# ZencashOfficial/ginger-lib

Hardware: AMD Instinct MI355X
Metric: MNT4-753 G1 MSM scalar-muls/sec + 2^n NTT ms at 1/2/4/8 MI355X (higher is better)
Workload: dtype u32 (29-bit limbs of 753-bit Montgomery residues, 64-bit accumulators)

## Files before the change

ginger-lib_amd/asmgen/build.py:

```python
import json
import os
import subprocess
import sys

from . import g1_reduce, g1_xyzz, g2_rounds, microbench, ntt_pass
from .isa import module_text

LLVM = os.environ.get("GH_LLVM_BIN", "/opt/rocm/lib/llvm/bin")

P4 = 0x1c4c62d92c41110229022eee2cdadb7f997505b8fafed5eb7e8f96c97d87307fdb925e8a0ed8d99d124d9a15af79db117e776f218059db80f0da5cb537e38685acce9767254a4638810719ac425f0e39d54522cdd119f5e9063de245e8001
P6 = 0x1c4c62d92c41110229022eee2cdadb7f997505b8fafed5eb7e8f96c97d87307fdb925e8a0ed8d99d124d9a15af79db26c5c28c859a99b3eebca9429212636b9dff97634993aa4d6c381bc3f0057974ea099170fa13a4fd90776e240000001
R = 1 << 754


def programs():
    progs = [
        g1_xyzz.build("gh_asm_acc_g1_p4", P4, R % P4),
        g1_xyzz.build("gh_asm_acc_g1_p6", P6, R % P6),
        g1_xyzz.build("gh_asm_acc_g1_p4_pw", P4, R % P4, persistent=True),
        g1_xyzz.build("gh_asm_acc_g1_p6_pw", P6, R % P6, persistent=True),
        g1_reduce.build("gh_asm_red_g1_p4", P4, R % P4),
        g1_reduce.build("gh_asm_red_g1_p6", P6, R % P6),
    ]
    c2 = g2_rounds.Cfg(2, 13, P4, R % P4)
    c3 = g2_rounds.Cfg(3, 11, P6, R % P6)
    c1a = g2_rounds.Cfg(1, 1, P4, R % P4)
    c1b = g2_rounds.Cfg(1, 1, P6, R % P6)
    for tag, cfg in (("f2", c2), ("f3", c3), ("f1p4", c1a), ("f1p6", c1b)):
        for fwd in (True, False):
            for r0 in (True, False):
                progs.append(g2_rounds.build("gh_asm_aff_%s_%s_%s" % (tag, "fwd" if fwd else "bwd", "r0" if r0 else "rn"), cfg, fwd, r0))
    for tag, prime in (("p4", P4), ("p6", P6)):
        for k in (6, 7, 8):
            progs.append(ntt_pass.build("gh_asm_ntt_%s_k%d" % (tag, k), prime, k))
    progs.append(microbench.build("gh_asm_mb_mulpair", P4))
    if os.environ.get("GH_ASM_DEBUG"):
        progs.append(g2_rounds.build("gh_asm_aff_f2_bwd_r0_dbg", c2, False, True, debug=True))
        for tag, prime in (("p4", P4), ("p6", P6)):
            progs.append(g1_xyzz.build("gh_asm_acc_g1_%s_dbg" % tag, prime, R % prime, debug=True))
            progs.append(g1_xyzz.build("gh_asm_acc_g1_%s_pw_dbg" % tag, prime, R % prime, persistent=True, debug=True))
    if os.environ.get("GH_ASM_VARIANTS"):
        progs += [g1_xyzz.build("gh_asm_acc_g1_p4_s1", P4, R % P4, split=1),
                  g1_xyzz.build("gh_asm_acc_g1_p4_s2", P4, R % P4, split=2),
                  g1_xyzz.build("gh_asm_acc_g1_p4_s1pf", P4, R % P4, split=1, prefetch=True)]
    return progs


def build(outdir):
    os.makedirs(outdir, exist_ok=True)
# ... 1 lines not shown
    text, infos = module_text(progs)
    s_path = os.path.join(outdir, "gh_asm.s")
    with open(s_path, "w") as f:
        f.write(text)
    o_path = os.path.join(outdir, "gh_asm.o")
    co_path = os.path.join(outdir, "gh_asm.hsaco")
    subprocess.run([os.path.join(LLVM, "clang"), "-x", "assembler", "-target", "amdgcn-amd-amdhsa", "-mcpu=gfx950",
                    "-c", s_path, "-o", o_path], check=True)
    subprocess.run([os.path.join(LLVM, "ld.lld"), "-shared", o_path, "-o", co_path], check=True)
    for p in progs:
        infos[p.name]["instructions"] = p.count()
        infos[p.name]["lds_bytes"] = p.lds_bytes
        infos[p.name]["scratch_bytes_per_lane"] = 0
        if getattr(p, "loop_labels", None):
            infos[p.name].update(g1_xyzz.update_counts(p))
    with open(os.path.join(outdir, "gh_asm.json"), "w") as f:
        json.dump(infos, f, indent=1, sort_keys=True)
    return co_path, infos


if __name__ == "__main__":
    co, infos = build(sys.argv[1] if len(sys.argv) > 1 else "build")
    print(co, json.dumps(infos))
```

ginger-lib_amd/asmgen/field.py:

```python
from .isa import Reg, V, S

NL = 26
LB = 29
LM = (1 << LB) - 1


ND = NL + 1
TOP_SHIFT = LB * (NL - 1)


class BoundError(ValueError):
    """a lazy routine was asked for operands whose columns, top limb or doubled limb do not fit the registers"""


class Bound:

    def __init__(self, k, slack=0):
        self.k, self.slack = k, slack

    def value(self, p):
        return self.k * p + self.slack

    def __repr__(self):
        return "Bound(%d p + 2^%.1f)" % (self.k, _log2(self.slack)) if self.slack else "Bound(%d p)" % self.k
# ... 428 lines not shown
            o = dst.sub(i) if i == NL - 1 else x
            if a is None:
                if i:
                    g.v_add_u32(o, t, c); yield
                else:
                    g.v_mov_b32(o, t); yield
            elif i:
                g.v_add3_u32(o, t, a.sub(i), c); yield
            else:
                g.v_add_u32(o, t, a.sub(0)); yield
            if i + 1 < NL:
                g.v_ashrrev_i32(c, LB, x); yield
                g.v_and_b32(dst.sub(i), S(self.s_lm), x); yield
        return res

    def zero_or_p_mask(self, ch, a, smask, stmp):
        g = self.g
        skip = g.uniq("zp_skip")
        g.v_cmp_eq_u32(smask, 0, a.sub(0))
        g.v_cmp_eq_u32(stmp, self.sP(0), a.sub(0))
        g.s_or_b64(smask, smask, stmp)
        g.s_cbranch_scc0(skip)
        run(self.is_zero_mask(ch, a, smask))
        x = ch.acc.lo()
        g.v_xor_b32(x, self.sP(0), a.sub(0))
        for i in range(1, NL):
            g.v_xor_b32(ch.t1, self.sP(i), a.sub(i))
            g.v_or_b32(x, x, ch.t1)
        g.v_cmp_eq_u32(stmp, 0, x)
        g.s_or_b64(smask, smask, stmp)
# ... 35 lines not shown
```

ginger-lib_amd/asmgen/ntt_pass.py:

```python
from .isa import Prog, V, S, VCC, EXEC, OFF, fix_hazards
from .field import FieldGen, Chain, run, NL, LB, LM

ARG_IN, ARG_OUT, ARG_TW, ARG_PRE, ARG_POST = 0, 8, 16, 24, 32
ARG_LOGN, ARG_LOGNS, ARG_INVERSE, ARG_POST_STRIDE, ARG_NWAVES = 40, 44, 48, 52, 56
ARG_BYTES = 64

S_KARG, S_WG = S(0, 2), S(2)
S_IN, S_OUT, S_TW, S_PRE, S_POST = S(4, 2), S(6, 2), S(8, 2), S(10, 2), S(12, 2)
S_LOGN, S_LOGNS, S_INVERSE, S_PSTRIDE, S_NWAVES = S(14), S(15), S(16), S(17), S(18)
S_LM, S_INV = 20, 21
S_P, S_NP = 24, 50
S_DUM, S_CAR, S_MASK = S(22, 2), S(76, 2), S(78, 2)
S_SSH, S_SH, S_NMASK, S_N, S_NSMASK, S_96, S_104, S_WAVE, S_T0, S_T1 = (S(80), S(81), S(82), S(83), S(84), S(85), S(86), S(87),
                                                                         S(88), S(89))

V_TID, V_LANE, V_TL, V_J, V_KK = V(0), V(1), V(2), V(3), V(4)
V_OFF = [V(5), V(6), V(7), V(8)]
V_IDX = [V(9), V(10), V(11), V(12)]
V_T = [V(13), V(14), V(15), V(16), V(17), V(18), V(19)]


def slot(i):
    return V(20 + NL * i, NL)


E = [slot(i) for i in range(4)]
TWA, TWB, M, D = slot(4), slot(5), slot(6), slot(7)
STAGE = [TWA, TWB, M, D]


def build(name, p, k):
    assert 4 <= k <= 8
    log_c = 8 - k
    g = Prog(name)
    for _ in range(5):
        g.add_arg(8, "ptr")
    for _ in range(6):
        g.add_arg(4, "val")
    assert g.kernarg_bytes == ARG_BYTES
    f = FieldGen(g, p, S_P, S_NP, S_INV, S_LM)
    ch = Chain(V(228, 2), V(230), V(231), S_DUM, S_CAR)
    L_END, L_GO = g.uniq("end"), g.uniq("go")

    def load_fp(dst, voff, sbase):
        for q in range(NL // 2):
            g.global_load_dwordx2(V(dst.idx + 2 * q, 2), voff, sbase, offset=8 * q)
# ... 29 lines not shown
                prev = w
            if lo + 1 < NL:
                g.v_lshl_or_b32(w, src.sub(lo + 1), LB - sh, prev)
                prev = w
            if lo + 2 < NL and 2 * LB - sh < 32:
                g.v_lshl_or_b32(w, src.sub(lo + 2), 2 * LB - sh, prev)
                prev = w
            assert prev is w

    def tw_offset(dst, e):
        g.v_sub_u32(V_T[6], S_N, e)
        g.v_and_b32(V_T[6], S_NMASK, V_T[6])
        g.v_cndmask_b32(dst, e, V_T[6], S_T0X)
        g.v_mul_lo_u32(dst, dst, S_104)

    def butterfly(x, y, tw):
        if tw is None:
            run(f.sub(ch, x, y, D))
            run(f.add_mod(ch, x, y))
            run(f.copy(y, D))
        else:
            run(f.mul(ch, y, tw, M, D, dst=D))
            run(f.sub(ch, x, D, y))
            run(f.add_mod(ch, x, D))

    def times(x, tw):
        run(f.mul(ch, x, tw, M, tw, dst=x))

    S_T0X = S(90, 2)

    g.s_load_dwordx8(S(4, 8), S_KARG, 0)
    g.s_load_dwordx8(S(12, 8), S_KARG, 32)
    f.load_constants()
    g.s_mov_b32(S_96, 96)
    g.s_mov_b32(S_104, 104)
    g.v_and_b32(V_LANE, 63, V_TID)
    g.v_lshrrev_b32(V_T[0], 6, V_TID)
    g.v_readfirstlane_b32(S_WAVE, V_T[0])
    g.s_lshl_b32(S_T0, S_WG, 2)
    g.s_add_u32(S_WAVE, S_WAVE, S_T0)
    g.s_waitcnt(lgkmcnt=0)
    g.s_cmp_lt_u32(S_WAVE, S_NWAVES)
    g.s_cbranch_scc1(L_GO)
    g.s_endpgm()
    g.label(L_GO)
    g.s_sub_u32(S_SSH, S_LOGN, k)
    g.s_sub_u32(S_SH, S_SSH, S_LOGNS)
    g.s_lshl_b32(S_N, 1, S_LOGN)
# ... 20 lines not shown
        load_raw(STAGE[a], V_OFF[a])
    for a in range(4):
        g.s_waitcnt(vmcnt=6 * (3 - a))
        unpack(E[a], STAGE[a])

    L_NOPRE = g.uniq("nopre")
    S_JMP = S(92, 2)
    g.s_cmp_eq_u64(S_PRE, 0)
    g.s_cbranch_scc0(g_pre := g.uniq("pre"))
    g.long_branch(L_NOPRE, S_JMP)
    g.label(g_pre)
    for a in range(4):
        g.v_mul_lo_u32(V_OFF[a], V_IDX[a], S_104)
    load_fp(TWA, V_OFF[0], S_PRE)
    for a in range(4):
        cur, nxt = (TWA, TWB) if a % 2 == 0 else (TWB, TWA)
        if a + 1 < 4:
            load_fp(nxt, V_OFF[a + 1], S_PRE)
            g.s_waitcnt(vmcnt=NL // 2)
        else:
            g.s_waitcnt(vmcnt=0)
        times(E[a], cur)
    g.label(L_NOPRE)


    inl = [k - 2, k - 1]
    V_BP, V_E, V_REV = V_T[4], V_T[5], V_T[3]
    S_T2 = S(94)
    g.v_bfrev_b32(V_REV, V_TL)
    g.v_lshrrev_b32(V_REV, 32 - (k - 2), V_REV)
    for beta in range(k - 1, -1, -1):
        last = beta == 0
        if beta in inl:
            b = inl.index(beta)
            swap_q = None
        else:
            b = 0 if inl[0] > inl[1] else 1
            swap_q = beta + log_c
        pairs = [(0, 2), (1, 3)] if b == 1 else [(0, 1), (2, 3)]
        g.s_add_u32(S_T1, S_SH, beta)
        g.s_add_u32(S_T2, S_SSH, beta)
        g.v_lshlrev_b32(V_E, S_T1, V_KK)
        tws = [TWA]
        if beta <= k - 2:
            nrev = k - 2 - beta
            if nrev > 0:
                g.v_and_b32(V_T[0], (1 << nrev) - 1, V_REV)
# ... 24 lines not shown
            inl[b] = beta
        g.s_waitcnt(vmcnt=0)
        for n, (x, y) in enumerate(pairs):
            tw = tws[min(n, len(tws) - 1)]
            if beta == k - 1 or (beta == k - 2 and n == 0):
                L_FULL, L_NEXT = g.uniq("full"), g.uniq("next")
                g.s_cmp_eq_u32(S_LOGNS, 0)
                g.s_cbranch_scc0(L_FULL)
                butterfly(E[x], E[y], None)
                g.long_branch(L_NEXT, S_JMP)
                g.label(L_FULL)
                butterfly(E[x], E[y], tw)
                g.label(L_NEXT)
            else:
                butterfly(E[x], E[y], tw)
    g.v_sub_u32(V_T[0], V_J, V_KK)
    g.v_lshlrev_b32(V_T[0], k, V_T[0])
    g.v_add_u32(V_T[0], V_T[0], V_KK)
    g.v_lshlrev_b32(V_T[1], 2, V_TL)
    g.v_bfrev_b32(V_T[1], V_T[1])
    g.v_lshrrev_b32(V_T[1], 32 - k, V_T[1])
    for a in range(4):
        t_low = (((a >> 0) & 1) << inl[0]) | (((a >> 1) & 1) << inl[1])
        rev = int(format(t_low, "0%db" % k)[::-1], 2)
        g.v_or_b32(V_IDX[a], rev, V_T[1])
        g.v_lshlrev_b32(V_IDX[a], S_LOGNS, V_IDX[a])
        g.v_add_u32(V_IDX[a], V_IDX[a], V_T[0])
    L_STORE = g.uniq("store")
    g.s_cmp_eq_u64(S_POST, 0)
    g.s_cbranch_scc0(g_post := g.uniq("post"))
    g.long_branch(L_STORE, S_JMP)
    g.label(g_post)
    for a in range(4):
        g.v_mul_lo_u32(V_OFF[a], V_IDX[a], S_PSTRIDE)
    load_fp(TWA, V_OFF[0], S_POST)
    for a in range(4):
        cur, nxt = (TWA, TWB) if a % 2 == 0 else (TWB, TWA)
        if a + 1 < 4:
            load_fp(nxt, V_OFF[a + 1], S_POST)
            g.s_waitcnt(vmcnt=NL // 2)
        else:
            g.s_waitcnt(vmcnt=0)
        times(E[a], cur)
    g.label(L_STORE)
    for a in range(4):
        g.v_mul_lo_u32(V_OFF[a], V_IDX[a], S_96)
    for a in range(4):
        pack(STAGE[a], E[a])
        for q in range(6):
            g.global_store_dwordx4(V_OFF[a], V(STAGE[a].idx + 4 * q, 4), S_OUT, offset=16 * q)
    g.s_endpgm()
    g.label(L_END)
    g.s_endpgm()
    g.hazard_nops = fix_hazards(g)
    return g
```

ginger-lib_amd/csrc/asm_kernels.h:

```cpp
#pragma once
#include "runtime.h"

namespace gh_asm {

struct AccTask {
    uint32_t beg, cnt;
    uint64_t dst;
};
static_assert(sizeof(AccTask) == 16, "the kernel reads one dwordx4 per task");

bool enabled();

int acc_g1_launch(int prime, const void* bases, const uint32_t* sorted, const AccTask* tasks, const void* salts,
                  uint32_t n_tasks, uint32_t* tile_counter, hipStream_t st);
int acc_stamps_read(uint32_t* out_words, size_t cap_words, uint32_t* n_records);

struct RedArgs {
    const void* items;
    void* out;
    void* slabs;
    uint32_t* flag;
    uint32_t count, valid, segs, L, n_programs, pad;
};
static_assert(sizeof(RedArgs) == 56, "argument block of gh_asm_red_g1_*");
// ... 15 lines not shown
};
static_assert(sizeof(AffArgs) == 88, "argument block of gh_asm_aff_*");

bool aff_enabled();
bool aff_g1_enabled();
int aff_launch(int kind, bool fwd, bool r0, const AffArgs& a, uint32_t waves, hipStream_t st);

struct NttAsmArgs {
    const void* in;
    void* out;
    const void* tw;
    const void* pre;
    const void* post;
    uint32_t log_n, log_ns, inverse;
    uint32_t post_stride;
    uint32_t n_waves, pad;
};
static_assert(sizeof(NttAsmArgs) == 64, "argument block of gh_asm_ntt_*");

bool ntt_enabled();
bool ntt_supported(int log_n, int k);
int ntt_pass_launch(int prime, int k, const NttAsmArgs& a, hipStream_t st);

int measure_fpmul_peak(double* products_per_s, hipStream_t st);
int kernel_resources(const char* which, uint32_t* scratch, uint32_t* vgprs, uint32_t* lds);

}
```

ginger-lib_amd/csrc/asm_kernels.hip:

```cpp
#include "asm_kernels.h"
#include <stdio.h>
#include <stdlib.h>
#include <string.h>
#include <vector>

extern "C" const unsigned char gh_asm_hsaco[];
extern "C" const unsigned char gh_asm_hsaco_end[];

namespace gh_asm {

using gh_rt::g;
using gh_rt::g_err;
using gh_rt::env_int;

namespace {
constexpr int NTT_ASM_KMIN = 6, NTT_ASM_KMAX = 8;
struct State {
    bool tried = false;
    hipModule_t mod = nullptr;
    hipFunction_t acc_g1[2] = {nullptr, nullptr};
    hipFunction_t acc_g1_pw[2] = {nullptr, nullptr};
    hipFunction_t acc_g1_dbg[2][2] = {};
    uint32_t* stamps[2] = {nullptr, nullptr};
    size_t stamps_cap[2] = {0, 0};
    uint32_t stamps_n = 0;
    int stamps_last = 1;
    hipFunction_t red_g1[2] = {nullptr, nullptr};
    hipFunction_t aff[4][2][2] = {};
    hipFunction_t mb_mulpair = nullptr;
    hipFunction_t ntt[2][3] = {};
};
State s;

int load_locked() {
    if (s.tried) return s.mod ? GH_OK : GH_E_HIP;
    s.tried = true;
    const size_t bytes = (size_t)(gh_asm_hsaco_end - gh_asm_hsaco);
    if (bytes < 64 || memcmp(gh_asm_hsaco, "\177ELF", 4) != 0) {
        g_err = "assembly code object missing from the library (build/gh_asm.hsaco was not embedded)";
        return GH_E_HIP;
    }
    hipModule_t m = nullptr;
    hipError_t e;
    static std::vector<char> override_co;
    if (const char* path = getenv("GH_ASM_HSACO")) {
// ... 51 lines not shown
        }
    }
    static const char* kinds[4] = {"f2", "f3", "f1p4", "f1p6"};
    for (int t = 0; t < 4; t++)
        for (int fw = 0; fw < 2; fw++)
            for (int r0 = 0; r0 < 2; r0++) {
                char nm[64];
                snprintf(nm, sizeof nm, "gh_asm_aff_%s_%s_%s", kinds[t], fw ? "fwd" : "bwd", r0 ? "r0" : "rn");
                e = hipModuleGetFunction(&s.aff[t][fw][r0], m, nm);
                if (e != hipSuccess) {
                    g_err = std::string("hipModuleGetFunction(") + nm + ") failed: " + hipGetErrorString(e);
                    hipModuleUnload(m);
                    return GH_E_HIP;
                }
            }
    for (int f = 0; f < 2; f++)
        for (int k = NTT_ASM_KMIN; k <= NTT_ASM_KMAX; k++) {
            char nm[64];
            snprintf(nm, sizeof nm, "gh_asm_ntt_p%d_k%d", f ? 6 : 4, k);
            e = hipModuleGetFunction(&s.ntt[f][k - NTT_ASM_KMIN], m, nm);
            if (e != hipSuccess) {
                g_err = std::string("hipModuleGetFunction(") + nm + ") failed: " + hipGetErrorString(e);
                hipModuleUnload(m);
                return GH_E_HIP;
            }
        }
    e = hipModuleGetFunction(&s.mb_mulpair, m, "gh_asm_mb_mulpair");
    if (e != hipSuccess) {
        g_err = std::string("hipModuleGetFunction(gh_asm_mb_mulpair) failed: ") + hipGetErrorString(e);
        hipModuleUnload(m);
        return GH_E_HIP;
    }
    s.mod = m;
    g.at_shutdown.push_back([] {
        if (s.mod) hipModuleUnload(s.mod);
        for (uint32_t* b : s.stamps) if (b) (void)hipFree(b);
        s = State();
    });
    return GH_OK;
}
}
// ... 126 lines not shown
        return GH_E_UNSUPPORTED;
    }
    if (int rc = load_locked()) return rc;
    AffArgs args = a;
    size_t size = sizeof args;
    void* extra[] = {HIP_LAUNCH_PARAM_BUFFER_POINTER, &args, HIP_LAUNCH_PARAM_BUFFER_SIZE, &size, HIP_LAUNCH_PARAM_END};
    HIPCHK(hipModuleLaunchKernel(s.aff[tower][fwd ? 1 : 0][r0 ? 1 : 0], waves / 4, 1, 1, 256, 1, 1, 0, st, nullptr, extra));
    return GH_OK;
}

bool ntt_enabled() {
    static const bool on = env_int("GH_NTT_ASM", 1) != 0;
    return on;
}

bool ntt_supported(int log_n, int k) { return k >= NTT_ASM_KMIN && k <= NTT_ASM_KMAX && log_n >= 8 && log_n <= 25 && k <= log_n; }

int ntt_pass_launch(int prime, int k, const NttAsmArgs& a, hipStream_t st) {
    if (!ntt_supported((int)a.log_n, k) || a.log_ns + (uint32_t)k > a.log_n || a.n_waves != (1u << (a.log_n - 8)) ||
        (a.post_stride != 0 && a.post_stride != 104)) {
        g_err = "internal: NTT pass outside the assembly kernel's range";
        return GH_E_UNSUPPORTED;
    }
    if (int rc = load_locked()) return rc;
    NttAsmArgs args = a;
    size_t size = sizeof args;
    void* extra[] = {HIP_LAUNCH_PARAM_BUFFER_POINTER, &args, HIP_LAUNCH_PARAM_BUFFER_SIZE, &size, HIP_LAUNCH_PARAM_END};
    HIPCHK(hipModuleLaunchKernel(s.ntt[prime == 6 ? 1 : 0][k - NTT_ASM_KMIN], (a.n_waves + 3) / 4, 1, 1, 256, 1, 1, 0, st, nullptr, extra));
    return GH_OK;
}

int measure_fpmul_peak(double* products_per_s, hipStream_t st) {
    if (int rc = load_locked()) return rc;
    const uint32_t iters = 200, blocks = (uint32_t)g.num_cus * 2u;
    struct { uint32_t iters, pad; } args = {iters, 0};
    size_t size = sizeof args;
    void* extra[] = {HIP_LAUNCH_PARAM_BUFFER_POINTER, &args, HIP_LAUNCH_PARAM_BUFFER_SIZE, &size, HIP_LAUNCH_PARAM_END};
    hipEvent_t e0, e1;
    HIPCHK(hipEventCreate(&e0));
    HIPCHK(hipEventCreate(&e1));
    float best = 0;
    for (int rep = 0; rep < 4; rep++) {
        HIPCHK(hipEventRecord(e0, st));
// ... 14 lines not shown
    if (int rc = load_locked()) return rc;
    hipFunction_t f = nullptr;
    const std::string w = which ? which : "";
    if (w == "g1_acc_p4") f = s.acc_g1[0];
    else if (w == "g1_acc_p6") f = s.acc_g1[1];
    else if (w == "g1_acc_p4_pw") f = s.acc_g1_pw[0];
    else if (w == "g1_acc_p6_pw") f = s.acc_g1_pw[1];
    else if (w == "g1_red_p4") f = s.red_g1[0];
    else if (w == "g1_red_p6") f = s.red_g1[1];
    else if (w == "g2_f2_fwd_r0") f = s.aff[0][1][1];
    else if (w == "g2_f2_bwd_r0") f = s.aff[0][0][1];
    else if (w == "g2_f2_bwd_rn") f = s.aff[0][0][0];
    else if (w == "g2_f3_fwd_r0") f = s.aff[1][1][1];
    else if (w == "g2_f3_bwd_r0") f = s.aff[1][0][1];
    else if (w == "g2_f3_bwd_rn") f = s.aff[1][0][0];
    else if (w == "ntt_p4_k8") f = s.ntt[0][2];
    else if (w == "ntt_p6_k8") f = s.ntt[1][2];
    else { g_err = "unknown kernel name"; return GH_E_BAD_ARG; }
    int v = 0;
    HIPCHK(hipFuncGetAttribute(&v, HIP_FUNC_ATTRIBUTE_LOCAL_SIZE_BYTES, f));
    if (scratch) *scratch = (uint32_t)v;
    HIPCHK(hipFuncGetAttribute(&v, HIP_FUNC_ATTRIBUTE_NUM_REGS, f));
    if (vgprs) *vgprs = (uint32_t)v;
    HIPCHK(hipFuncGetAttribute(&v, HIP_FUNC_ATTRIBUTE_SHARED_SIZE_BYTES, f));
    if (lds) *lds = (uint32_t)v;
    return GH_OK;
}

}
```

ginger-lib_amd/csrc/fp29.h:

```cpp
#pragma once
#include <stdint.h>
#include "constants_gen.h"

#if defined(__HIPCC__)
#define GH_HD __host__ __device__ __forceinline__
#define GH_HD_NOINLINE __host__ __device__ __attribute__((noinline))
#define GH_UNROLL _Pragma("unroll")
#else
#define GH_HD inline
#define GH_HD_NOINLINE __attribute__((noinline))
#define GH_UNROLL
#endif

namespace gh {

constexpr int NL = 26;
constexpr int LB = 29;
constexpr uint32_t LM = (1u << LB) - 1;

struct Fp {
    uint32_t l[NL];
};

struct P4 {
// ... 370 lines not shown
template <class P> GH_HD bool fp_is_zero_or_p(const Fp& a) {
    if (a.l[0] != 0 && a.l[0] != P::P[0]) return false;
    uint32_t z = 0, e = 0;
    GH_UNROLL for (int i = 0; i < NL; i++) {
        z |= a.l[i];
        e |= a.l[i] ^ P::P[i];
    }
    return z == 0 || e == 0;
}
template <class P> GH_HD Fp fp_lazy_one() {
    Fp d3 = fp_zero();
    d3.l[3] = 1;
    Fp c = fp_mul27<P>(fp_const<P>(P::R2I), d3);
    fp_cond_sub<P>(c);
    return c;
}

constexpr int FP_INV_BATCHES = 61;

template <class P> GH_HD Fp fp_inv_plain(const Fp& x) {
    int32_t d[NL], e[NL], f[NL], g[NL];
    GH_UNROLL for (int i = 0; i < NL; i++) { d[i] = 0; e[i] = 0; f[i] = (int32_t)P::P[i]; g[i] = (int32_t)x.l[i]; }
    e[0] = 1;
    int32_t zeta = -1;
    const uint32_t pinv = (0u - P::INV) & LM;
#if defined(__HIP_DEVICE_COMPILE__)
#pragma nounroll
#endif
    for (int it = 0; it < FP_INV_BATCHES; it++) {
        uint32_t u = 1, v = 0, q = 0, r = 1, fl = (uint32_t)f[0], gl = (uint32_t)g[0];
// ... 244 lines not shown
```

ginger-lib_amd/csrc/ntt.hip:

```cpp
#include "runtime.h"
#include "ntt_kernels.h"
#include "host_math.h"
#include "asm_kernels.h"

namespace gh_rt {
using namespace gh;

template <class P> struct FieldConsts;
template <> struct FieldConsts<P6> {
    static constexpr int two_adicity = GH_P6_TWO_ADICITY;
    static const uint64_t* root_m() { static const uint64_t v[12] = GH_P6_ROOT_M_64; return v; }
    static const uint64_t* gen_m() { static const uint64_t v[12] = GH_P6_GEN17_M_64; return v; }
};
template <> struct FieldConsts<P4> {
    static constexpr int two_adicity = GH_P4_TWO_ADICITY;
    static const uint64_t* root_m() { static const uint64_t v[12] = GH_P4_ROOT_M_64; return v; }
    static const uint64_t* gen_m() { static const uint64_t v[12] = GH_P4_GEN17_M_64; return v; }
};

template <class P> int build_pow_table(Fp* tab, int log_n, const Fp& first, Fp base) {
    HIPCHK(hipMemcpyAsync(tab, &first, sizeof(Fp), hipMemcpyHostToDevice, g.stream));
    HIPCHK(hipStreamSynchronize(g.stream));
    for (int s = 0; s < log_n; s++) {
        uint32_t half = 1u << s;
        hipLaunchKernelGGL((pow_table_step_kernel<P>), dim3((half + 255) / 256), dim3(256), 0, g.stream, tab, half, base);
        base = fp_sqr<P>(base);
    }
    HIPCHK(hipGetLastError());
    return GH_OK;
}

template <class P> int build_table_checked(DevMem& t, int log_n, const Fp& first, const Fp& base) {
    int rc;
    if ((rc = t.alloc(((size_t)1 << log_n) * sizeof(Fp))) || (rc = build_pow_table<P>(t.as<Fp>(), log_n, first, base))) return rc;
    if (hipStreamSynchronize(g.stream) != hipSuccess) { g_err = "building a domain table failed"; return GH_E_HIP; }
    return GH_OK;
}

template <class P> int get_domain(int fidx, int log_n, bool need_coset, bool need_coset_inv, Domain** out) {
    auto it = g.domains[fidx].find(log_n);
    const size_t N = (size_t)1 << log_n;
    if (it == g.domains[fidx].end()) {
        Domain d;
        d.log_n = log_n;
        Fp w = fp_from_abi<P>(reinterpret_cast<const uint32_t*>(FieldConsts<P>::root_m()));
        for (int i = log_n; i < FieldConsts<P>::two_adicity; i++) w = fp_sqr<P>(w);
        Fp n_int = fp_one<P>();
        for (int i = 0; i < log_n; i++) n_int = fp_dbl<P>(n_int);
        d.size_inv = host_fp_inv<P>(n_int);
        DevMem scratch, tw, size_inv;
        int rc;
        if ((rc = scratch.alloc(N * 96)) || (rc = build_table_checked<P>(tw, log_n, fp_one<P>(), w)) || (rc = size_inv.alloc(128))) return rc;
        HIPCHK(hipMemcpy(size_inv.get(), &d.size_inv, sizeof(Fp), hipMemcpyHostToDevice));
        d.scratch = (uint32_t*)scratch.release();
        d.tw = (Fp*)tw.release();
        d.d_size_inv = (Fp*)size_inv.release();
        it = g.domains[fidx].emplace(log_n, d).first;
    }
    Domain& d = it->second;
    if (need_coset && !d.coset) {
        Fp gen = fp_from_abi<P>(reinterpret_cast<const uint32_t*>(FieldConsts<P>::gen_m()));
        DevMem t;
        if (int rc = build_table_checked<P>(t, log_n, fp_one<P>(), gen)) return rc;
        d.coset = (Fp*)t.release();
    }
    if (need_coset_inv && !d.coset_inv) {
        Fp gen = fp_from_abi<P>(reinterpret_cast<const uint32_t*>(FieldConsts<P>::gen_m()));
        Fp gi = host_fp_inv<P>(gen);
        DevMem t;
        if (int rc = build_table_checked<P>(t, log_n, d.size_inv, gi)) return rc;
        d.coset_inv = (Fp*)t.release();
    }
    *out = &d;
    return GH_OK;
}

template <class P> int fft_run(int fidx, void* d_data, uint32_t log_n, uint32_t flags, bool sync = true) {
    if ((int)log_n >= FieldConsts<P>::two_adicity) {
        g_err = "domain exceeds the field's 2-adicity";
        return GH_E_UNSUPPORTED;
    }
    g.last_fft_ms = 0;
    if (log_n == 0) return GH_OK;
    const bool inverse = flags & GH_FFT_INVERSE, coset = flags & GH_FFT_COSET;
    Domain* d;
    int rc = get_domain<P>(fidx, (int)log_n, coset && !inverse, coset && inverse, &d);
    if (rc) return rc;
    const int P_ = ((int)log_n + NTT_MAX_LOGR - 1) / NTT_MAX_LOGR;
    int ks[8];
    {
        int base = (int)log_n / P_, rem = (int)log_n % P_;
        for (int s = 0; s < P_; s++) ks[s] = base + (s < rem ? 1 : 0);
    }
    static bool attr_set[2] = {false, false};
    if (!attr_set[fidx]) {
        HIPCHK(hipFuncSetAttribute(reinterpret_cast<const void*>(&ntt_pass_kernel<P>),
                                   hipFuncAttributeMaxDynamicSharedMemorySize, NL * 4 * NTT_MAX_TILE));
        attr_set[fidx] = true;
    }
    if (P_ >= 3 && (P_ & 1) && !d->scratch2 && !d->scratch2_failed) {
        DevMem s2;
        if (s2.alloc(((size_t)96) << log_n)) {
            (void)hipGetLastError();
            d->scratch2_failed = true;
        }
        d->scratch2 = (uint32_t*)s2.release();
    }
    const bool three = P_ >= 3 && (P_ & 1) && d->scratch2;
    uint32_t* bufs[2] = {(uint32_t*)d_data, d->scratch};
    int cur = 0, log_ns = 0;
    static const bool ntt_asm = gh_asm::ntt_enabled();
    HIPCHK(hipEventRecord(g.ev[4], g.stream));
    for (int s = 0; s < P_; s++) {
        NttPassArgs A;
        A.in = bufs[cur];
        A.out = bufs[cur ^ 1];
        if (three) {
            if (s == 0) { A.in = (uint32_t*)d_data; A.out = d->scratch; }
            else if (s == 1) { A.in = d->scratch; A.out = d->scratch2; }
            else if (s == 2) { A.in = d->scratch2; A.out = (uint32_t*)d_data; }
        }
        A.tw = d->tw;
        A.pre = (s == 0 && coset && !inverse) ? d->coset : nullptr;
        A.post = nullptr;
        A.has_post_scalar = 0;
        A.post_scalar = d->size_inv;
        if (s == P_ - 1 && inverse) {
            if (coset) A.post = d->coset_inv; else A.has_post_scalar = 1;
        }
        A.log_n = (int)log_n;
        A.k = ks[s];
        A.log_ns = log_ns;
        int log_c = (int)log_n - ks[s];
        if (log_c > NTT_LOG_TILE - ks[s]) log_c = NTT_LOG_TILE - ks[s];
        A.log_c = log_c;
        A.inverse = inverse ? 1 : 0;
        const int E = 1 << (ks[s] + log_c);
        int threads = E / 2;
        if (threads < 64) threads = 64;
        const unsigned grid = 1u << ((int)log_n - ks[s] - log_c);
        if (ntt_asm && gh_asm::ntt_supported((int)log_n, ks[s])) {
            gh_asm::NttAsmArgs q;
            q.in = A.in; q.out = A.out; q.tw = A.tw; q.pre = A.pre;
            q.post = A.post ? (const void*)A.post : (A.has_post_scalar ? (const void*)d->d_size_inv : nullptr);
            q.post_stride = A.post ? 104u : 0u;
            q.log_n = log_n; q.log_ns = (uint32_t)log_ns; q.inverse = (uint32_t)A.inverse;
            q.n_waves = 1u << (log_n - 8); q.pad = 0;
            if ((rc = gh_asm::ntt_pass_launch(std::is_same<P, P6>::value ? 6 : 4, ks[s], q, g.stream))) return rc;
        } else {
            hipLaunchKernelGGL((ntt_pass_kernel<P>), dim3(grid), dim3(threads), (size_t)NL * 4 * E, g.stream, A);
        }
        if (three && s < 3) cur = s == 2 ? 0 : 1;
        else cur ^= 1;
        log_ns += ks[s];
    }
    HIPCHK(hipGetLastError());
    if (cur == 1) HIPCHK(hipMemcpyAsync(d_data, d->scratch, ((size_t)96) << log_n, hipMemcpyDeviceToDevice, g.stream));
    HIPCHK(hipEventRecord(g.ev[5], g.stream));
    if (sync) {
        HIPCHK(hipStreamSynchronize(g.stream));
        HIPCHK(hipEventElapsedTime(&g.last_fft_ms, g.ev[4], g.ev[5]));
    }
    return GH_OK;
// ... 97 lines not shown
    if ((int)log_n >= FieldConsts<P>::two_adicity) { g_err = "domain exceeds the field's 2-adicity"; return GH_E_UNSUPPORTED; }
    const size_t N = (size_t)1 << log_n;
    const Fp tau = fp_from_abi<P>(reinterpret_cast<const uint32_t*>(tau12));
    Fp t_size = tau;
    for (uint32_t i = 0; i < log_n; i++) t_size = fp_sqr<P>(t_size);
    const dim3 grid((unsigned)((N + 255) / 256)), blk(256);
    Fp one_tab = fp_one<P>();
    const Fp* tw = nullptr;
    DevMem tw1;
    if (log_n == 0) {
        if (int rc = tw1.alloc(sizeof(Fp))) return rc;
        HIPCHK(hipMemcpy(tw1.get(), &one_tab, sizeof(Fp), hipMemcpyHostToDevice));
        tw = tw1.as<Fp>();
    } else {
        Domain* d;
        int rc = get_domain<P>(fidx, (int)log_n, false, false, &d);
        if (rc) return rc;
        tw = d->tw;
    }
    int rc = GH_OK;
    if (fp_eq(t_size, fp_one<P>())) {
        hipLaunchKernelGGL((lagrange_kernel<P, 0>), grid, blk, 0, g.stream, (uint32_t*)d_out, tw, N, tau, fp_zero());
    } else {
        Fp n_int = fp_one<P>();
        for (uint32_t i = 0; i < log_n; i++) n_int = fp_dbl<P>(n_int);
        const Fp l0 = fp_mul<P>(fp_sub<P>(t_size, fp_one<P>()), host_fp_inv<P>(n_int));
        hipLaunchKernelGGL((lagrange_kernel<P, 1>), grid, blk, 0, g.stream, (uint32_t*)d_out, tw, N, tau, l0);
        rc = batch_inverse_t<P>(d_out, N);
        if (!rc) hipLaunchKernelGGL((lagrange_kernel<P, 2>), grid, blk, 0, g.stream, (uint32_t*)d_out, tw, N, tau, l0);
    }
    hipError_t e = hipGetLastError();
    if (e == hipSuccess) e = hipStreamSynchronize(g.stream);
    if (!rc && e != hipSuccess) { g_err = std::string("lagrange coefficients: ") + hipGetErrorString(e); rc = GH_E_HIP; }
// ... 45 lines not shown
```

ginger-lib_amd/csrc/runtime.h:

```cpp
#pragma once
#include <hip/hip_runtime.h>
#include <stdint.h>
#include <stdio.h>
#include <stdlib.h>
#include <functional>
#include <map>
#include <mutex>
#include <string>
#include <vector>
#include "../../include/ginger_hip.h"
#include "fp29.h"
#include "msm_plan.h"

struct gh_poseidon;
namespace gh { struct Mnt4G1; struct Mnt4G2; struct Mnt6G1; struct Mnt6G2; }

namespace gh_rt {

template <class T> void dev_free(T*& p) {
    if (p) (void)hipFree(p);
    p = nullptr;
}

struct Domain {
    int log_n = 0;
    gh::Fp* tw = nullptr;
    gh::Fp* coset = nullptr;
    gh::Fp* coset_inv = nullptr;
    gh::Fp size_inv;
    gh::Fp* d_size_inv = nullptr;
    uint32_t* scratch = nullptr;
    uint32_t* scratch2 = nullptr;
    bool scratch2_failed = false;
    void release() { dev_free(tw); dev_free(coset); dev_free(coset_inv); dev_free(d_size_inv); dev_free(scratch); dev_free(scratch2); }
};

struct DevBuf {
    void* p = nullptr;
    size_t cap = 0;
};

struct Ctx {
    bool ready = false;
    int device = 0;
    int num_cus = 256;
    hipStream_t stream = nullptr;
    hipStream_t stream_acc = nullptr;
    hipStream_t stream_red = nullptr;
    hipStream_t stream_acc2 = nullptr;
// ... 171 lines not shown
```

Measured before the change: 54.74 million.

## Add lazy-reduction NTT pass kernels with mul27 twiddles and deferred final reduction

```diff
diff --git a/ginger-lib_amd/asmgen/build.py b/ginger-lib_amd/asmgen/build.py
--- a/ginger-lib_amd/asmgen/build.py
+++ b/ginger-lib_amd/asmgen/build.py
@@ -33,6 +33,7 @@
     for tag, prime in (("p4", P4), ("p6", P6)):
         for k in (6, 7, 8):
             progs.append(ntt_pass.build("gh_asm_ntt_%s_k%d" % (tag, k), prime, k))
+            progs.append(ntt_pass.build("gh_asm_ntt_%s_k%d_lz" % (tag, k), prime, k, lazy=True))
     progs.append(microbench.build("gh_asm_mb_mulpair", P4))
     if os.environ.get("GH_ASM_DEBUG"):
         progs.append(g2_rounds.build("gh_asm_aff_f2_bwd_r0_dbg", c2, False, True, debug=True))
@@ -64,6 +65,8 @@
         infos[p.name]["scratch_bytes_per_lane"] = 0
         if getattr(p, "loop_labels", None):
             infos[p.name].update(g1_xyzz.update_counts(p))
+        if getattr(p, "ntt_counts", None):
+            infos[p.name].update({"ntt_" + k: v for k, v in p.ntt_counts.items()})
     with open(os.path.join(outdir, "gh_asm.json"), "w") as f:
         json.dump(infos, f, indent=1, sort_keys=True)
     return co_path, infos
diff --git a/ginger-lib_amd/asmgen/field.py b/ginger-lib_amd/asmgen/field.py
--- a/ginger-lib_amd/asmgen/field.py
+++ b/ginger-lib_amd/asmgen/field.py
@@ -466,6 +466,47 @@
                 g.v_and_b32(dst.sub(i), S(self.s_lm), x); yield
         return res
 
+    def lazy_add(self, ch, a, b, dst, ba, bb):
+        g = self.g
+        ba, bb = _bound(ba), _bound(bb)
+        self._caps(ba), self._caps(bb)
+        res = Bound(ba.k + bb.k, ba.slack + bb.slack)
+        self._caps(res)
+        x, c = ch.t0, ch.t1
+        for i in range(NL):
+            o = dst.sub(i) if i == NL - 1 else x
+            if i:
+                g.v_add3_u32(o, a.sub(i), b.sub(i), c); yield
+            else:
+                g.v_add_u32(o, a.sub(0), b.sub(0)); yield
+            if i + 1 < NL:
+                g.v_lshrrev_b32(c, LB, x); yield
+                g.v_and_b32(dst.sub(i), S(self.s_lm), x); yield
+        return res
+
+    def top_quotient_bound(self, bx):
+        qmax = self._caps(bx)[NL - 1] // (self.pl[NL - 1] + 1)
+        return Bound(1, (qmax + 1) << TOP_SHIFT)
+
+    def reduce_top(self, ch, x, bx, s_invc):
+        g = self.g
+        res = self.top_quotient_bound(bx)
+        acc, nq = ch.acc, ch.t1
+        g.v_cvt_f64_u32(acc, x.sub(NL - 1)); yield
+        g.v_add_f64(acc, acc, "0.5"); yield
+        g.v_mul_f64(acc, acc, s_invc); yield
+        g.v_cvt_u32_f64(nq, acc); yield
+        g.v_sub_u32(nq, 0, nq); yield
+        for i in range(NL):
+            g.v_mad_i64_i32(acc, ch.sdum, nq, self.sP(i), 0 if i == 0 else acc); yield
+            g.v_mad_u64_u32(acc, ch.sdum, x.sub(i), 1, acc); yield
+            if i + 1 < NL:
+                g.v_and_b32(x.sub(i), S(self.s_lm), acc.lo()); yield
+                g.v_ashrrev_i64(acc, LB, acc); yield
+            else:
+                g.v_mov_b32(x.sub(i), acc.lo()); yield
+        return res
+
     def zero_or_p_mask(self, ch, a, smask, stmp):
         g = self.g
         skip = g.uniq("zp_skip")
diff --git a/ginger-lib_amd/asmgen/ntt_pass.py b/ginger-lib_amd/asmgen/ntt_pass.py
--- a/ginger-lib_amd/asmgen/ntt_pass.py
+++ b/ginger-lib_amd/asmgen/ntt_pass.py
@@ -1,13 +1,13 @@
 from .isa import Prog, V, S, VCC, EXEC, OFF, fix_hazards
-from .field import FieldGen, Chain, run, NL, LB, LM
+from .field import FieldGen, Chain, Bound, BoundError, run, runv, NL, LB, LM, TOP_SHIFT
 
 ARG_IN, ARG_OUT, ARG_TW, ARG_PRE, ARG_POST = 0, 8, 16, 24, 32
-ARG_LOGN, ARG_LOGNS, ARG_INVERSE, ARG_POST_STRIDE, ARG_NWAVES = 40, 44, 48, 52, 56
+ARG_LOGN, ARG_LOGNS, ARG_INVERSE, ARG_POST_STRIDE, ARG_NWAVES, ARG_LAZY_OUT = 40, 44, 48, 52, 56, 60
 ARG_BYTES = 64
 
 S_KARG, S_WG = S(0, 2), S(2)
 S_IN, S_OUT, S_TW, S_PRE, S_POST = S(4, 2), S(6, 2), S(8, 2), S(10, 2), S(12, 2)
-S_LOGN, S_LOGNS, S_INVERSE, S_PSTRIDE, S_NWAVES = S(14), S(15), S(16), S(17), S(18)
+S_LOGN, S_LOGNS, S_INVERSE, S_PSTRIDE, S_NWAVES, S_LAZY_OUT = S(14), S(15), S(16), S(17), S(18), S(19)
 S_LM, S_INV = 20, 21
 S_P, S_NP = 24, 50
 S_DUM, S_CAR, S_MASK = S(22, 2), S(76, 2), S(78, 2)
@@ -29,7 +29,20 @@
 STAGE = [TWA, TWB, M, D]
 
 
-def build(name, p, k):
+LAZY_GROWTH = 2
+LAZY_SLACK_STEP = 1 << 734
+
+
+def lazy_in_bound(f):
+    return f.top_quotient_bound(lazy_stage_bound(f, 8, LAZY_GROWTH, Bound(1, 32 << TOP_SHIFT)))
+
+
+def lazy_stage_bound(f, j, growth=LAZY_GROWTH, b_in=None):
+    b_in = lazy_in_bound(f) if b_in is None else b_in
+    return Bound(1 + growth * j, b_in.slack + j * LAZY_SLACK_STEP)
+
+
+def build(name, p, k, lazy=False, growth=LAZY_GROWTH):
     assert 4 <= k <= 8
     log_c = 8 - k
     g = Prog(name)
@@ -89,24 +102,62 @@
         g.v_cndmask_b32(dst, e, V_T[6], S_T0X)
         g.v_mul_lo_u32(dst, dst, S_104)
 
+    def fits(b, limit):
+        if b.value(p) > limit.value(p):
+            raise BoundError("%s: a value can reach %r, declared %r" % (name, b, limit))
+
+    def lazy_butterfly(x, y, tw):
+        bx = by = cur[0]
+        n0 = g.count()
+        if tw is None:
+            if by.value(p) > 2 * p:
+                by = runv(f.reduce_top(ch, y, by, S_INVC))
+            bd = runv(f.lazy_diff(ch, x, [(y, 1)], 1, D, bx, [by]))
+            bs = runv(f.lazy_add(ch, x, y, x, bx, by))
+            run(f.copy(y, D))
+        else:
+            bt = runv(f.mul27(ch, y, tw, M, by, Bound(1), r=D))
+            bd = runv(f.lazy_diff(ch, x, [(D, 1)], 1, y, bx, [bt]))
+            bs = runv(f.lazy_add(ch, x, D, x, bx, bt))
+            counts["butterfly"] = g.count() - n0
+        fits(bd, cur[1])
+        fits(bs, cur[1])
+
     def butterfly(x, y, tw):
-        if tw is None:
+        if lazy:
+            lazy_butterfly(x, y, tw)
+        elif tw is None:
             run(f.sub(ch, x, y, D))
             run(f.add_mod(ch, x, y))
             run(f.copy(y, D))
         else:
+            n0 = g.count()
             run(f.mul(ch, y, tw, M, D, dst=D))
             run(f.sub(ch, x, D, y))
             run(f.add_mod(ch, x, D))
+            counts["butterfly"] = g.count() - n0
 
     def times(x, tw):
+        if lazy:
+            return runv(f.mul27(ch, x, tw, M, cur[0], Bound(1), r=x))
         run(f.mul(ch, x, tw, M, tw, dst=x))
+
+    counts = {}
+    g.ntt_counts = counts
+    S_INVC = S(96, 2)
+    if lazy:
+        b_in = lazy_in_bound(f)
+        cur = [b_in, b_in]
 
     S_T0X = S(90, 2)
 
     g.s_load_dwordx8(S(4, 8), S_KARG, 0)
     g.s_load_dwordx8(S(12, 8), S_KARG, 32)
     f.load_constants()
+    if lazy:
+        lo, hi = f.invc_bits()
+        g.s_mov_b32(S(S_INVC.idx), lo)
+        g.s_mov_b32(S(S_INVC.idx + 1), hi)
     g.s_mov_b32(S_96, 96)
     g.s_mov_b32(S_104, 104)
     g.v_and_b32(V_LANE, 63, V_TID)
@@ -157,14 +208,16 @@
         g.v_mul_lo_u32(V_OFF[a], V_IDX[a], S_104)
     load_fp(TWA, V_OFF[0], S_PRE)
     for a in range(4):
-        cur, nxt = (TWA, TWB) if a % 2 == 0 else (TWB, TWA)
+        cur_tw, nxt = (TWA, TWB) if a % 2 == 0 else (TWB, TWA)
         if a + 1 < 4:
             load_fp(nxt, V_OFF[a + 1], S_PRE)
             g.s_waitcnt(vmcnt=NL // 2)
         else:
             g.s_waitcnt(vmcnt=0)
-        times(E[a], cur)
+        b_pre = times(E[a], cur_tw)
     g.label(L_NOPRE)
+    if lazy:
+        fits(b_pre, b_in)
 
 
     inl = [k - 2, k - 1]
@@ -174,6 +227,8 @@
     g.v_lshrrev_b32(V_REV, 32 - (k - 2), V_REV)
     for beta in range(k - 1, -1, -1):
         last = beta == 0
+        if lazy:
+            cur[1] = lazy_stage_bound(f, k - beta, growth, b_in)
         if beta in inl:
             b = inl.index(beta)
             swap_q = None
@@ -228,6 +283,8 @@
                 g.label(L_NEXT)
             else:
                 butterfly(E[x], E[y], tw)
+        if lazy:
+            cur[0] = cur[1]
     g.v_sub_u32(V_T[0], V_J, V_KK)
     g.v_lshlrev_b32(V_T[0], k, V_T[0])
     g.v_add_u32(V_T[0], V_T[0], V_KK)
@@ -249,14 +306,35 @@
         g.v_mul_lo_u32(V_OFF[a], V_IDX[a], S_PSTRIDE)
     load_fp(TWA, V_OFF[0], S_POST)
     for a in range(4):
-        cur, nxt = (TWA, TWB) if a % 2 == 0 else (TWB, TWA)
+        cur_tw, nxt = (TWA, TWB) if a % 2 == 0 else (TWB, TWA)
         if a + 1 < 4:
             load_fp(nxt, V_OFF[a + 1], S_POST)
             g.s_waitcnt(vmcnt=NL // 2)
         else:
             g.s_waitcnt(vmcnt=0)
-        times(E[a], cur)
-    g.label(L_STORE)
+        b_post = times(E[a], cur_tw)
+    if lazy:
+        L_RED, L_CS = g.uniq("red"), g.uniq("cs")
+        fits(b_post, b_in)
+        g.long_branch(L_CS, S_JMP)
+        g.label(L_STORE)
+        n0 = g.count()
+        for a in range(4):
+            fits(runv(f.reduce_top(ch, E[a], cur[0], S_INVC)), b_in)
+        counts["reduce_top"] = (g.count() - n0) // 4
+        g.label(L_CS)
+        assert b_in.value(p) < 2 * p
+        g.s_cmp_eq_u32(S_LAZY_OUT, 0)
+        g.s_cbranch_scc1(L_RED)
+        g.long_branch(L_OUT := g.uniq("out"), S_JMP)
+        g.label(L_RED)
+        n0 = g.count()
+        for a in range(4):
+            run(f.cond_sub(ch, E[a], D, E[a]))
+        counts["cond_sub"] = (g.count() - n0) // 4
+        g.label(L_OUT)
+    else:
+        g.label(L_STORE)
     for a in range(4):
         g.v_mul_lo_u32(V_OFF[a], V_IDX[a], S_96)
     for a in range(4):
diff --git a/ginger-lib_amd/csrc/asm_kernels.h b/ginger-lib_amd/csrc/asm_kernels.h
--- a/ginger-lib_amd/csrc/asm_kernels.h
+++ b/ginger-lib_amd/csrc/asm_kernels.h
@@ -53,13 +53,15 @@
     const void* post;
     uint32_t log_n, log_ns, inverse;
     uint32_t post_stride;
-    uint32_t n_waves, pad;
+    uint32_t n_waves;
+    uint32_t lazy_out;
 };
 static_assert(sizeof(NttAsmArgs) == 64, "argument block of gh_asm_ntt_*");
 
 bool ntt_enabled();
+bool ntt_lazy_enabled();
 bool ntt_supported(int log_n, int k);
-int ntt_pass_launch(int prime, int k, const NttAsmArgs& a, hipStream_t st);
+int ntt_pass_launch(int prime, int k, bool lazy, const NttAsmArgs& a, hipStream_t st);
 
 int measure_fpmul_peak(double* products_per_s, hipStream_t st);
 int kernel_resources(const char* which, uint32_t* scratch, uint32_t* vgprs, uint32_t* lds);
diff --git a/ginger-lib_amd/csrc/asm_kernels.hip b/ginger-lib_amd/csrc/asm_kernels.hip
--- a/ginger-lib_amd/csrc/asm_kernels.hip
+++ b/ginger-lib_amd/csrc/asm_kernels.hip
@@ -28,7 +28,7 @@
     hipFunction_t red_g1[2] = {nullptr, nullptr};
     hipFunction_t aff[4][2][2] = {};
     hipFunction_t mb_mulpair = nullptr;
-    hipFunction_t ntt[2][3] = {};
+    hipFunction_t ntt[2][2][3] = {};
 };
 State s;
 
@@ -110,17 +110,18 @@
                     return GH_E_HIP;
                 }
             }
-    for (int f = 0; f < 2; f++)
-        for (int k = NTT_ASM_KMIN; k <= NTT_ASM_KMAX; k++) {
-            char nm[64];
-            snprintf(nm, sizeof nm, "gh_asm_ntt_p%d_k%d", f ? 6 : 4, k);
-            e = hipModuleGetFunction(&s.ntt[f][k - NTT_ASM_KMIN], m, nm);
-            if (e != hipSuccess) {
-                g_err = std::string("hipModuleGetFunction(") + nm + ") failed: " + hipGetErrorString(e);
-                hipModuleUnload(m);
-                return GH_E_HIP;
+    for (int lz = 0; lz < 2; lz++)
+        for (int f = 0; f < 2; f++)
+            for (int k = NTT_ASM_KMIN; k <= NTT_ASM_KMAX; k++) {
+                char nm[64];
+                snprintf(nm, sizeof nm, "gh_asm_ntt_p%d_k%d%s", f ? 6 : 4, k, lz ? "_lz" : "");
+                e = hipModuleGetFunction(&s.ntt[lz][f][k - NTT_ASM_KMIN], m, nm);
+                if (e != hipSuccess) {
+                    g_err = std::string("hipModuleGetFunction(") + nm + ") failed: " + hipGetErrorString(e);
+                    hipModuleUnload(m);
+                    return GH_E_HIP;
+                }
             }
-        }
     e = hipModuleGetFunction(&s.mb_mulpair, m, "gh_asm_mb_mulpair");
     if (e != hipSuccess) {
         g_err = std::string("hipModuleGetFunction(gh_asm_mb_mulpair) failed: ") + hipGetErrorString(e);
@@ -277,11 +278,16 @@
     return on;
 }
 
+bool ntt_lazy_enabled() {
+    static const bool on = env_int("GH_NTT_LAZY", 1) != 0;
+    return on;
+}
+
 bool ntt_supported(int log_n, int k) { return k >= NTT_ASM_KMIN && k <= NTT_ASM_KMAX && log_n >= 8 && log_n <= 25 && k <= log_n; }
 
-int ntt_pass_launch(int prime, int k, const NttAsmArgs& a, hipStream_t st) {
+int ntt_pass_launch(int prime, int k, bool lazy, const NttAsmArgs& a, hipStream_t st) {
     if (!ntt_supported((int)a.log_n, k) || a.log_ns + (uint32_t)k > a.log_n || a.n_waves != (1u << (a.log_n - 8)) ||
-        (a.post_stride != 0 && a.post_stride != 104)) {
+        (a.post_stride != 0 && a.post_stride != 104) || a.lazy_out > (lazy ? 1u : 0u)) {
         g_err = "internal: NTT pass outside the assembly kernel's range";
         return GH_E_UNSUPPORTED;
     }
@@ -289,7 +295,7 @@
     NttAsmArgs args = a;
     size_t size = sizeof args;
     void* extra[] = {HIP_LAUNCH_PARAM_BUFFER_POINTER, &args, HIP_LAUNCH_PARAM_BUFFER_SIZE, &size, HIP_LAUNCH_PARAM_END};
-    HIPCHK(hipModuleLaunchKernel(s.ntt[prime == 6 ? 1 : 0][k - NTT_ASM_KMIN], (a.n_waves + 3) / 4, 1, 1, 256, 1, 1, 0, st, nullptr, extra));
+    HIPCHK(hipModuleLaunchKernel(s.ntt[lazy ? 1 : 0][prime == 6 ? 1 : 0][k - NTT_ASM_KMIN], (a.n_waves + 3) / 4, 1, 1, 256, 1, 1, 0, st, nullptr, extra));
     return GH_OK;
 }
 
@@ -334,8 +340,10 @@
     else if (w == "g2_f3_fwd_r0") f = s.aff[1][1][1];
     else if (w == "g2_f3_bwd_r0") f = s.aff[1][0][1];
     else if (w == "g2_f3_bwd_rn") f = s.aff[1][0][0];
-    else if (w == "ntt_p4_k8") f = s.ntt[0][2];
-    else if (w == "ntt_p6_k8") f = s.ntt[1][2];
+    else if (w == "ntt_p4_k8") f = s.ntt[0][0][2];
+    else if (w == "ntt_p6_k8") f = s.ntt[0][1][2];
+    else if (w == "ntt_p4_k8_lz") f = s.ntt[1][0][2];
+    else if (w == "ntt_p6_k8_lz") f = s.ntt[1][1][2];
     else { g_err = "unknown kernel name"; return GH_E_BAD_ARG; }
     int v = 0;
     HIPCHK(hipFuncGetAttribute(&v, HIP_FUNC_ATTRIBUTE_LOCAL_SIZE_BYTES, f));
diff --git a/ginger-lib_amd/csrc/fp29.h b/ginger-lib_amd/csrc/fp29.h
--- a/ginger-lib_amd/csrc/fp29.h
+++ b/ginger-lib_amd/csrc/fp29.h
@@ -408,6 +408,43 @@
     Fp c = fp_mul27<P>(fp_const<P>(P::R2I), d3);
     fp_cond_sub<P>(c);
     return c;
+}
+
+GH_HD Fp fp_lazy_add(const Fp& a, const Fp& b) {
+    Fp t;
+    uint32_t cy = 0;
+    GH_UNROLL for (int i = 0; i < NL; i++) {
+        const uint32_t x = a.l[i] + b.l[i] + cy;
+        t.l[i] = i == NL - 1 ? x : x & LM;
+        cy = x >> LB;
+    }
+    return t;
+}
+template <class P> GH_HD Fp fp_reduce_top(const Fp& x) {
+    const int64_t q = x.l[NL - 1] / (P::P[NL - 1] + 1u);
+    Fp r;
+    int64_t acc = 0;
+    GH_UNROLL for (int i = 0; i < NL; i++) {
+        acc += (int64_t)x.l[i] - q * (int64_t)P::P[i];
+        r.l[i] = i == NL - 1 ? (uint32_t)acc : (uint32_t)acc & LM;
+        acc >>= LB;
+    }
+    return r;
+}
+template <class P> GH_HD void fp_ntt_lazy_butterfly(Fp& x, Fp& y, const Fp& v_rd) {
+    const Fp t = fp_mul27<P>(y, v_rd);
+    y = fp_lazy_sub<P, 1>(x, t);
+    x = fp_lazy_add(x, t);
+}
+template <class P> GH_HD void fp_ntt_lazy_butterfly_one(Fp& x, Fp& y, bool reduce_y) {
+    const Fp t = reduce_y ? fp_reduce_top<P>(y) : y;
+    y = fp_lazy_sub<P, 1>(x, t);
+    x = fp_lazy_add(x, t);
+}
+template <class P> GH_HD Fp fp_ntt_lazy_finish(const Fp& x, bool lazy_out) {
+    Fp r = fp_reduce_top<P>(x);
+    if (!lazy_out) fp_cond_sub<P>(r);
+    return r;
 }
 
 constexpr int FP_INV_BATCHES = 61;
diff --git a/ginger-lib_amd/csrc/ntt.hip b/ginger-lib_amd/csrc/ntt.hip
--- a/ginger-lib_amd/csrc/ntt.hip
+++ b/ginger-lib_amd/csrc/ntt.hip
@@ -37,39 +37,63 @@
     return GH_OK;
 }
 
-template <class P> int get_domain(int fidx, int log_n, bool need_coset, bool need_coset_inv, Domain** out) {
+template <class P> Fp lazy_table_factor() {
+    Fp d = fp_one<P>();
+    for (int i = 0; i < LB; i++) d = fp_dbl<P>(d);
+    return d;
+}
+
+struct DomainNeeds {
+    unsigned tw = 0, coset = 0, coset_inv = 0, size_inv = 0;
+};
+
+template <class P> int get_domain(int fidx, int log_n, const DomainNeeds& need, Domain** out) {
     auto it = g.domains[fidx].find(log_n);
     const size_t N = (size_t)1 << log_n;
     if (it == g.domains[fidx].end()) {
         Domain d;
         d.log_n = log_n;
-        Fp w = fp_from_abi<P>(reinterpret_cast<const uint32_t*>(FieldConsts<P>::root_m()));
-        for (int i = log_n; i < FieldConsts<P>::two_adicity; i++) w = fp_sqr<P>(w);
         Fp n_int = fp_one<P>();
         for (int i = 0; i < log_n; i++) n_int = fp_dbl<P>(n_int);
         d.size_inv = host_fp_inv<P>(n_int);
-        DevMem scratch, tw, size_inv;
-        int rc;
-        if ((rc = scratch.alloc(N * 96)) || (rc = build_table_checked<P>(tw, log_n, fp_one<P>(), w)) || (rc = size_inv.alloc(128))) return rc;
-        HIPCHK(hipMemcpy(size_inv.get(), &d.size_inv, sizeof(Fp), hipMemcpyHostToDevice));
+        DevMem scratch;
+        if (int rc = scratch.alloc(N * 96)) return rc;
         d.scratch = (uint32_t*)scratch.release();
-        d.tw = (Fp*)tw.release();
-        d.d_size_inv = (Fp*)size_inv.release();
         it = g.domains[fidx].emplace(log_n, d).first;
     }
     Domain& d = it->second;
-    if (need_coset && !d.coset) {
-        Fp gen = fp_from_abi<P>(reinterpret_cast<const uint32_t*>(FieldConsts<P>::gen_m()));
-        DevMem t;
-        if (int rc = build_table_checked<P>(t, log_n, fp_one<P>(), gen)) return rc;
-        d.coset = (Fp*)t.release();
-    }
-    if (need_coset_inv && !d.coset_inv) {
-        Fp gen = fp_from_abi<P>(reinterpret_cast<const uint32_t*>(FieldConsts<P>::gen_m()));
-        Fp gi = host_fp_inv<P>(gen);
-        DevMem t;
-        if (int rc = build_table_checked<P>(t, log_n, d.size_inv, gi)) return rc;
-        d.coset_inv = (Fp*)t.release();
+    for (int f = 0; f < 2; f++) {
+        const bool missing = (((need.tw >> f) & 1) && !d.tw[f]) || (((need.size_inv >> f) & 1) && !d.d_size_inv[f]) ||
+                             (((need.coset >> f) & 1) && !d.coset[f]) || (((need.coset_inv >> f) & 1) && !d.coset_inv[f]);
+        if (!missing) continue;
+        const Fp one = f ? lazy_table_factor<P>() : fp_one<P>();
+        const Fp size_inv = f ? fp_mul<P>(d.size_inv, one) : d.size_inv;
+        if (((need.tw >> f) & 1) && !d.tw[f]) {
+            Fp w = fp_from_abi<P>(reinterpret_cast<const uint32_t*>(FieldConsts<P>::root_m()));
+            for (int i = log_n; i < FieldConsts<P>::two_adicity; i++) w = fp_sqr<P>(w);
+            DevMem t;
+            if (int rc = build_table_checked<P>(t, log_n, one, w)) return rc;
+            d.tw[f] = (Fp*)t.release();
+        }
+        if (((need.size_inv >> f) & 1) && !d.d_size_inv[f]) {
+            DevMem t;
+            if (int rc = t.alloc(128)) return rc;
+            HIPCHK(hipMemcpy(t.get(), &size_inv, sizeof(Fp), hipMemcpyHostToDevice));
+            d.d_size_inv[f] = (Fp*)t.release();
+        }
+        if (((need.coset >> f) & 1) && !d.coset[f]) {
+            Fp gen = fp_from_abi<P>(reinterpret_cast<const uint32_t*>(FieldConsts<P>::gen_m()));
+            DevMem t;
+            if (int rc = build_table_checked<P>(t, log_n, one, gen)) return rc;
+            d.coset[f] = (Fp*)t.release();
+        }
+        if (((need.coset_inv >> f) & 1) && !d.coset_inv[f]) {
+            Fp gen = fp_from_abi<P>(reinterpret_cast<const uint32_t*>(FieldConsts<P>::gen_m()));
+            Fp gi = host_fp_inv<P>(gen);
+            DevMem t;
+            if (int rc = build_table_checked<P>(t, log_n, size_inv, gi)) return rc;
+            d.coset_inv[f] = (Fp*)t.release();
+        }
     }
     *out = &d;
     return GH_OK;
@@ -83,15 +107,28 @@
     g.last_fft_ms = 0;
     if (log_n == 0) return GH_OK;
     const bool inverse = flags & GH_FFT_INVERSE, coset = flags & GH_FFT_COSET;
-    Domain* d;
-    int rc = get_domain<P>(fidx, (int)log_n, coset && !inverse, coset && inverse, &d);
-    if (rc) return rc;
     const int P_ = ((int)log_n + NTT_MAX_LOGR - 1) / NTT_MAX_LOGR;
     int ks[8];
     {
         int base = (int)log_n / P_, rem = (int)log_n % P_;
         for (int s = 0; s < P_; s++) ks[s] = base + (s < rem ? 1 : 0);
     }
+    static const bool ntt_asm = gh_asm::ntt_enabled(), ntt_lazy = gh_asm::ntt_lazy_enabled();
+    int kind[8];
+    DomainNeeds need;
+    for (int s = 0; s < P_; s++) {
+        kind[s] = ntt_asm && gh_asm::ntt_supported((int)log_n, ks[s]) ? (ntt_lazy ? 2 : 1) : 0;
+        const unsigned f = kind[s] == 2 ? 2u : 1u;
+        need.tw |= f;
+        if (s == 0 && coset && !inverse) need.coset |= f;
+        if (s == P_ - 1 && inverse) {
+            if (coset) need.coset_inv |= f;
+            else if (kind[s]) need.size_inv |= f;
+        }
+    }
+    Domain* d;
+    int rc = get_domain<P>(fidx, (int)log_n, need, &d);
+    if (rc) return rc;
     static bool attr_set[2] = {false, false};
     if (!attr_set[fidx]) {
         HIPCHK(hipFuncSetAttribute(reinterpret_cast<const void*>(&ntt_pass_kernel<P>),
@@ -109,7 +146,6 @@
     const bool three = P_ >= 3 && (P_ & 1) && d->scratch2;
     uint32_t* bufs[2] = {(uint32_t*)d_data, d->scratch};
     int cur = 0, log_ns = 0;
-    static const bool ntt_asm = gh_asm::ntt_enabled();
     HIPCHK(hipEventRecord(g.ev[4], g.stream));
     for (int s = 0; s < P_; s++) {
         NttPassArgs A;
@@ -120,13 +156,14 @@
             else if (s == 1) { A.in = d->scratch; A.out = d->scratch2; }
             else if (s == 2) { A.in = d->scratch2; A.out = (uint32_t*)d_data; }
         }
-        A.tw = d->tw;
-        A.pre = (s == 0 && coset && !inverse) ? d->coset : nullptr;
+        const int tf = kind[s] == 2 ? 1 : 0;
+        A.tw = d->tw[tf];
+        A.pre = (s == 0 && coset && !inverse) ? d->coset[tf] : nullptr;
         A.post = nullptr;
         A.has_post_scalar = 0;
         A.post_scalar = d->size_inv;
         if (s == P_ - 1 && inverse) {
-            if (coset) A.post = d->coset_inv; else A.has_post_scalar = 1;
+            if (coset) A.post = d->coset_inv[tf]; else A.has_post_scalar = 1;
         }
         A.log_n = (int)log_n;
         A.k = ks[s];
@@ -139,14 +176,15 @@
         int threads = E / 2;
         if (threads < 64) threads = 64;
         const unsigned grid = 1u << ((int)log_n - ks[s] - log_c);
-        if (ntt_asm && gh_asm::ntt_supported((int)log_n, ks[s])) {
+        if (kind[s]) {
             gh_asm::NttAsmArgs q;
             q.in = A.in; q.out = A.out; q.tw = A.tw; q.pre = A.pre;
-            q.post = A.post ? (const void*)A.post : (A.has_post_scalar ? (const void*)d->d_size_inv : nullptr);
+            q.post = A.post ? (const void*)A.post : (A.has_post_scalar ? (const void*)d->d_size_inv[tf] : nullptr);
             q.post_stride = A.post ? 104u : 0u;
             q.log_n = log_n; q.log_ns = (uint32_t)log_ns; q.inverse = (uint32_t)A.inverse;
-            q.n_waves = 1u << (log_n - 8); q.pad = 0;
-            if ((rc = gh_asm::ntt_pass_launch(std::is_same<P, P6>::value ? 6 : 4, ks[s], q, g.stream))) return rc;
+            q.n_waves = 1u << (log_n - 8);
+            q.lazy_out = (kind[s] == 2 && s + 1 < P_ && kind[s + 1] == 2) ? 1u : 0u;
+            if ((rc = gh_asm::ntt_pass_launch(std::is_same<P, P6>::value ? 6 : 4, ks[s], kind[s] == 2, q, g.stream))) return rc;
         } else {
             hipLaunchKernelGGL((ntt_pass_kernel<P>), dim3(grid), dim3(threads), (size_t)NL * 4 * E, g.stream, A);
         }
@@ -274,9 +312,11 @@
         tw = tw1.as<Fp>();
     } else {
         Domain* d;
-        int rc = get_domain<P>(fidx, (int)log_n, false, false, &d);
+        DomainNeeds need;
+        need.tw = 1;
+        int rc = get_domain<P>(fidx, (int)log_n, need, &d);
         if (rc) return rc;
-        tw = d->tw;
+        tw = d->tw[0];
     }
     int rc = GH_OK;
     if (fp_eq(t_size, fp_one<P>())) {
diff --git a/ginger-lib_amd/csrc/runtime.h b/ginger-lib_amd/csrc/runtime.h
--- a/ginger-lib_amd/csrc/runtime.h
+++ b/ginger-lib_amd/csrc/runtime.h
@@ -24,15 +24,18 @@
 
 struct Domain {
     int log_n = 0;
-    gh::Fp* tw = nullptr;
-    gh::Fp* coset = nullptr;
-    gh::Fp* coset_inv = nullptr;
+    gh::Fp* tw[2] = {nullptr, nullptr};
+    gh::Fp* coset[2] = {nullptr, nullptr};
+    gh::Fp* coset_inv[2] = {nullptr, nullptr};
     gh::Fp size_inv;
-    gh::Fp* d_size_inv = nullptr;
+    gh::Fp* d_size_inv[2] = {nullptr, nullptr};
     uint32_t* scratch = nullptr;
     uint32_t* scratch2 = nullptr;
     bool scratch2_failed = false;
-    void release() { dev_free(tw); dev_free(coset); dev_free(coset_inv); dev_free(d_size_inv); dev_free(scratch); dev_free(scratch2); }
+    void release() {
+        for (int f = 0; f < 2; f++) { dev_free(tw[f]); dev_free(coset[f]); dev_free(coset_inv[f]); dev_free(d_size_inv[f]); }
+        dev_free(scratch); dev_free(scratch2);
+    }
 };
 
 struct DevBuf {
```

Result: no change. 54.68 million (-0.1%).
